# afombravo/2FAST2Q

Measured on AMD Instinct MI355X. Metric: Mreads/sec matched (150 bp, 20 bp feature, m=1), higher is better.
Workload: dtype u64 (2-bit packed bases) / u8 qualities

## Files before the change

2fast2q_amd/csrc/f2q_count_kernels.h:

```cpp
#pragma once

#define F2Q_HIST_MAX 24576u
#define F2Q_HIST_RANGE 38912u

__device__ __forceinline__ unsigned long long wave_sum(unsigned long long v)
{
    for (int o = 32; o > 0; o >>= 1) v += __shfl_down(v, o, 64);
    return v;
}

__device__ __forceinline__ void flush_stats(const Accum &acc, unsigned long long st[5], unsigned long long *lds8,
                                            unsigned long long *slab_row)
{
    const uint32_t lane = threadIdx.x & 63u;
    if (threadIdx.x < 8) lds8[threadIdx.x] = 0;
    __syncthreads();
    for (int k = 0; k < 5; k++) {
        unsigned long long v = wave_sum(st[k]);
        if (lane == 0 && v) atomicAdd(&lds8[k], v);
    }
    __syncthreads();
    if (threadIdx.x < 5) {
        unsigned long long v = lds8[threadIdx.x];
        if (slab_row) gpw(slab_row)[threadIdx.x] = v;
// ... 278 lines not shown
    unsigned long long st[5] = {0, 0, 0, 0, 0};
    auto count_hit = [&](uint32_t idx) {
        if (USE_LDS) atomicAdd(&hist[idx], 1u);
        else acc_add(&acc.counts[idx], 1ull);
    };
    auto drain = [&](bool all) {
        __builtin_amdgcn_fence(__ATOMIC_ACQ_REL, "wavefront");
        const uint32_t tail = q_tail;
        while (all ? (tail != q_head) : (tail - q_head >= 64u)) {
            if (lane < tail - q_head) {
                const unsigned long long e = queue[(q_head + lane) % F2Q_V2_QCAP];
                uint32_t idx = 0;
                const int r = packed_near_decide(run, lib, lib.mpk[(uint32_t)(e >> 62)], e & ((1ull << 62) - 1ull),
                                                 qforced[(q_head + lane) % F2Q_V2_QCAP], idx);
                if (r == R_IMPERFECT || r == R_PERFECT) { count_hit(idx); st[2]++; } else st[3]++;
            }
            q_head += (tail - q_head < 64u) ? (tail - q_head) : 64u;
        }
        __builtin_amdgcn_fence(__ATOMIC_ACQ_REL, "wavefront");
    };
    for (uint32_t base = blockIdx.x * F2Q_V2_WAVES; base < pb.n_tiles; base += gridDim.x * F2Q_V2_WAVES) {
        const uint32_t tile = base + wave;
        if (tile < pb.n_tiles) {
            int res[4]; uint64_t key[4] = {0, 0, 0, 0}; uint32_t forced[4] = {0, 0, 0, 0}, npart[4] = {0, 0, 0, 0}, lv[4];
            {
                typedef uint32_t v2 __attribute__((ext_vector_type(2)));
                v2 len2 = {pb.rmax | (pb.rmax << 16), pb.rmax | (pb.rmax << 16)};
                if (pb.len) len2 = *(const v2 F2Q_GLOBAL *)(gp(pb.len) + (uint64_t)tile * F2Q_TILE + 4u * lane);
#pragma unroll
                for (int j = 0; j < 4; j++) {
                    lv[j] = ((j < 2 ? len2.x : len2.y) >> (16 * (j & 1))) & 0xFFFFu;
                    res[j] = lv[j] == F2Q_LEN_SKIP ? R_SKIP : ((int)(lv[j] & F2Q_LEN_MASK) < need) ? R_SLOW : R_NEAR;
                }
            }
            const auto qp = gp(pb.qual) + (uint64_t)tile * pb.wq * F2Q_TILE + 4u * lane;
            const auto bp = gp(pb.bases) + (uint64_t)tile * pb.wb * F2Q_TILE + 4u * lane;
            for (int w = 0; w < W; w++) {
                const FixedGeom g = fixed_geom_of(run, w);
                U4 brow[F2Q_MAXBROWS], qrow[F2Q_MAXQROWS];
#pragma unroll
                for (int r = 0; r < F2Q_MAXBROWS; r++) {
                    uint32_t row = (uint32_t)g.bw0 + (uint32_t)(r < g.nb ? r : g.nb - 1);
                    row = row < pb.wb ? row : pb.wb - 1u;
                    brow[r] = ld_u4<true>(bp + (uint64_t)row * F2Q_TILE);
                }
#pragma unroll
                for (int r = 0; r < F2Q_MAXQROWS; r++) {
                    uint32_t row = (uint32_t)g.qw0 + (uint32_t)(r < g.nq ? r : g.nq - 1);
                    row = row < pb.wq ? row : pb.wq - 1u;
                    qrow[r] = ld_u4<true>(qp + (uint64_t)row * F2Q_TILE);
                }
                uint32_t bad[4] = {0, 0, 0, 0};
                if (g.add_hi) {
#pragma unroll
                    for (int r = 0; r < F2Q_MAXQROWS; r++)
                        if (r < g.nq) fixed4_qrow(g, r, qrow[r], bad);
                }
#pragma unroll
                for (int j = 0; j < 4; j++) {
                    if (res[j] != R_NEAR || bad[j]) continue;
                    key[j] |= fixed4_key(g, brow, j) << (2u * (uint32_t)L * npart[j]);
                    if (lv[j] & F2Q_LEN_FLAG) forced[j] |= fixed4_flags(g, qrow, j) << ((uint32_t)L * npart[j]);
                    npart[j]++;
                }
            }
#pragma unroll
            for (int j = 0; j < 4; j++) {
                if (res[j] == R_SLOW) {
                    unsigned long long st2[5] = {0, 0, 0, 0, 0};
                    const Accum acc2 = acc; const PackedBlock pb2 = pb;
                    multi_slow(runp, libp, &acc2, &pb2, tile, 4u * lane + (uint32_t)j, (int)(lv[j] & F2Q_LEN_MASK), st2);
#pragma unroll
                    for (int k = 0; k < 5; k++) st[k] += st2[k];
                    res[j] = R_SKIP;
                } else if (res[j] == R_NEAR) {
                    st[0]++;
                    if (npart[j] == 0u) { res[j] = R_QFAIL; st[4]++; }
                    else if (forced[j]) res[j] = (!do_near || __popc(forced[j]) > run.miss) ? R_NONALIGNED : R_FORCED;
                }
            }
            for (int k = W; k >= 1; k--) {
                bool mine[4]; bool any = false;
#pragma unroll
                for (int j = 0; j < 4; j++) { mine[j] = res[j] == R_NEAR && npart[j] == (uint32_t)k; any |= mine[j]; }
                if (__ballot(any) == 0ull) continue;
                const PackedGroup &pk = lib.mpk[k - 1];
                const PackedPiece ex = pk.exact;
                const uint32_t ib = pk.ib, exm = (1u << ex.bits) - 1u;
                const uint64_t imask = (1ull << ib) - 1ull;
                if (pk.len == 0u) continue;
                uint32_t s[4];
#pragma unroll
                for (int j = 0; j < 4; j++) s[j] = packed_start(key[j], ex.bits);
                while (mine[0] | mine[1] | mine[2] | mine[3]) {
                    uint64_t v0[4], v1[4];
#pragma unroll
                    for (int j = 0; j < 4; j++)
                        if (mine[j]) { const Slot2 pr = packed_pair(ptab, ex.off + s[j]); v0[j] = pr.a; v1[j] = pr.b; }
#pragma unroll
                    for (int j = 0; j < 4; j++) {
                        if (!mine[j]) continue;
                        if (v0[j] == KEY_EMPTY) mine[j] = false;
                        else if ((v0[j] >> ib) == key[j]) { mine[j] = false; res[j] = R_PERFECT; count_hit((uint32_t)(v0[j] & imask)); }
                        else if (v1[j] == KEY_EMPTY) mine[j] = false;
                        else if ((v1[j] >> ib) == key[j]) { mine[j] = false; res[j] = R_PERFECT; count_hit((uint32_t)(v1[j] & imask)); }
                        else s[j] = (s[j] + 2u) & exm;
                    }
                }
            }
            uint32_t npush = 0;
#pragma unroll
            for (int j = 0; j < 4; j++) {
                if (res[j] == R_NEAR) { if (do_near) npush++; else res[j] = R_NONALIGNED; }
                else if (res[j] == R_FORCED) npush++;
                st[1] += (res[j] == R_PERFECT); st[3] += (res[j] == R_NONALIGNED);
            }
            {
                const unsigned long long b0 = __ballot(npush & 1u), b1 = __ballot(npush & 2u), b2 = __ballot(npush & 4u);
                uint32_t at = q_tail + __builtin_amdgcn_mbcnt_hi((uint32_t)(b0 >> 32), __builtin_amdgcn_mbcnt_lo((uint32_t)b0, 0u))
                              + 2u * __builtin_amdgcn_mbcnt_hi((uint32_t)(b1 >> 32), __builtin_amdgcn_mbcnt_lo((uint32_t)b1, 0u))
                              + 4u * __builtin_amdgcn_mbcnt_hi((uint32_t)(b2 >> 32), __builtin_amdgcn_mbcnt_lo((uint32_t)b2, 0u));
                q_tail += (uint32_t)__popcll(b0) + 2u * (uint32_t)__popcll(b1) + 4u * (uint32_t)__popcll(b2);
#pragma unroll
                for (int j = 0; j < 4; j++)
                    if (res[j] == R_NEAR || res[j] == R_FORCED) {
                        queue[at % F2Q_V2_QCAP] = key[j] | ((unsigned long long)(npart[j] - 1u) << 62);
                        qforced[at % F2Q_V2_QCAP] = forced[j];
                        at++;
                    }
            }
        }
        if (do_near) drain(false);
    }
    if (do_near) drain(true);
    __shared__ unsigned long long st_lds[8];
    flush_stats(acc, st, st_lds, acc.stat_slab ? acc.stat_slab + (uint64_t)blockIdx.x * 8u : nullptr);
    if (USE_LDS) {
        __syncthreads();
        auto row = gpw(acc.slab) + (uint64_t)blockIdx.x * nf;
        for (uint32_t i = tid; i < nf; i += F2Q_V2_THREADS) row[i] = hist[i];
    }
}

#define F2Q_LT_THREADS 1024
#define F2Q_LT_WAVES (F2Q_LT_THREADS / 64)

__device__ __forceinline__ U2 lds_u2(const uint32_t *p)
{
    typedef uint32_t v2 __attribute__((ext_vector_type(2)));
    const v2 v = *reinterpret_cast<const v2 *>(p);
    return U2{v.x, v.y};
}

__device__ __forceinline__ void lt_count(uint32_t *cnt, uint32_t slot, const Accum &acc, const LtDesc &lt)
{
    const uint32_t sh = (slot & 1u) << 4;
    const uint32_t old = atomicAdd(&cnt[slot >> 1], 1u << sh);
    if (((old >> sh) & 0xFFFFu) == 0x7FFFu) {
        atomicSub(&cnt[slot >> 1], 0x8000u << sh);
        acc_add(&acc.counts[gp(lt.feat_of)[slot]], 0x8000ull);
    }
}

template <int NQ, int NB, bool NEAR, bool A20, bool MW = false>
__global__ __launch_bounds__(F2Q_LT_THREADS) void k_count_fixed4_lds(const RunDev *__restrict__ runp,
                                                                     const LibDev *__restrict__ libp, PackedBlock pb,
                                                                     Accum acc)
{
    extern __shared__ uint32_t lt_smem[];
    constexpr uint32_t NT = NEAR ? 2u : 1u;
    uint32_t *tg = lt_smem;
    uint32_t *cnt = lt_smem + NT * F2Q_LT_SLOTS;
    const RunDev &run = *runp;
    const LibDev &lib = *libp;
    LtDesc lt = lib.lt;
    if (A20) { lt.hb0 = 20u; lt.hb1 = 20u; lt.len = 20u; }
    const uint32_t nf = lib.n_features;
    const uint32_t tid = threadIdx.x, lane = tid & 63u, wave = tid >> 6;
    {
        typedef uint32_t v4 __attribute__((ext_vector_type(4)));
        const v4 F2Q_GLOBAL *src = (const v4 F2Q_GLOBAL *)gp(lt.tags);
        v4 *dst = reinterpret_cast<v4 *>(tg);
        for (uint32_t i = tid; i < NT * F2Q_LT_SLOTS / 4u; i += F2Q_LT_THREADS) dst[i] = src[i];
        for (uint32_t i = tid; i < F2Q_LT_BUCKETS; i += F2Q_LT_THREADS) cnt[i] = 0;
    }
    __syncthreads();
    FixedGeom g = MW ? fixed_geom_at(0, run.n_iter * run.length, run.thr) : fixed_geom(run);
    if (A20) { g.L = 20; g.nq = 5; g.nb = 2; g.sh = 0; g.qm_first = 0x80808080u; g.qm_last = 0x80808080u; g.kmask = (1ull << 40) - 1ull; }
    const int need = g.st + g.L;
    uint32_t w_reads = 0, w_perfect = 0, w_imperfect = 0, w_qfail = 0;
    constexpr int QR = NQ ? NQ : F2Q_MAXQROWS, BR = NB ? NB : F2Q_MAXBROWS;
    constexpr bool PIPE = NQ != 0;

    struct Rows { U4 b[BR], q[QR]; uint32_t len01, len23; };
    const uint64_t q_stride = (uint64_t)pb.wq * F2Q_TILE, b_stride = (uint64_t)pb.wb * F2Q_TILE;
    const auto q_base = gp(pb.qual) + (uint64_t)g.qw0 * F2Q_TILE + 4u * lane;
    const auto b_base = gp(pb.bases) + (uint64_t)g.bw0 * F2Q_TILE + 4u * lane;
    const auto l_base = gp(pb.len) + 4u * lane;
    auto request_tile = [&](Rows &r, uint32_t t) {
        const auto qp = q_base + (uint64_t)t * q_stride;
        const auto bp = b_base + (uint64_t)t * b_stride;
#pragma unroll
        for (int i = 0; i < BR; i++) r.b[i] = ld_u4<true>(bp + (NB ? i : (i < g.nb ? i : g.nb - 1)) * F2Q_TILE);
#pragma unroll
        for (int i = 0; i < QR; i++) r.q[i] = ld_u4<true>(qp + (NQ ? i : (i < g.nq ? i : g.nq - 1)) * F2Q_TILE);
        typedef uint32_t v2 __attribute__((ext_vector_type(2)));
        const v2 lv = __builtin_nontemporal_load((const v2 F2Q_GLOBAL *)(l_base + (uint64_t)t * F2Q_TILE));
        r.len01 = lv.x; r.len23 = lv.y;
    };
    auto decide_tile = [&](const Rows &r) {
        uint32_t bad[4] = {0, 0, 0, 0};
        bool part_fail[4] = {false, false, false, false};
        if (MW && g.add_hi) {
#pragma unroll
            for (int j = 0; j < 4; j++) {
                const int pv = mw_part_verdict(fixed4_failbits(g, r.q, j), run.n_iter, run.length);
                bad[j] = pv == 2 ? 1u : 0u; part_fail[j] = pv == 1;
            }
        } else if (g.add_hi) {
            if (A20) {
#pragma unroll
                for (int i = 0; i < QR; i++) {
#pragma unroll
                    for (int j = 0; j < 4; j++) {
                        const uint32_t w = u4get(r.q[i], j) & 0x7F7F7F7Fu;
                        bad[j] |= (w + g.add_lo) & ~(w + g.add_hi);
                    }
                }
#pragma unroll
                for (int j = 0; j < 4; j++) bad[j] &= 0x80808080u;
            } else {
#pragma unroll
                for (int i = 0; i < QR; i++)
                    if (NQ || i < g.nq) fixed4_qrow(g, i, r.q[i], bad);
            }
        }
#pragma unroll
        for (int jp = 0; jp < 4; jp += 2) {
            LtProbe q[2]; U2 e[2][4]; uint32_t forced[2]; bool cand[2];
#pragma unroll
            for (int a = 0; a < 2; a++) {
                const int j = jp + a;
                const uint32_t l = ((j < 2 ? r.len01 : r.len23) >> (16 * (j & 1))) & 0xFFFFu;
                const bool live = l != F2Q_LEN_SKIP, qf = live && bad[j] != 0u;
                cand[a] = live && !qf && (int)(l & F2Q_LEN_MASK) >= need && !(MW && part_fail[j]);
                w_reads += (uint32_t)__popcll(__ballot(live));
                w_qfail += (uint32_t)__popcll(__ballot(qf));
                forced[a] = 0;
                if ((l & F2Q_LEN_FLAG) && cand[a]) forced[a] = fixed4_flags(g, r.q, j);
                uint64_t key = fixed4_key(g, r.b, j);
                if (MW && lt.mix) { key = mw_mix(key, lt.mix); if (forced[a]) forced[a] = mw_mix_mask(forced[a], lt.mix); }
                q[a] = lt_probe(lt, key);
#pragma unroll
                for (int k = 0; k < (NEAR ? 4 : 2); k++) e[a][k] = lds_u2(tg + (uint32_t)(k >> 1) * F2Q_LT_SLOTS + 2u * q[a].b[k]);
                if (!NEAR) { e[a][2] = U2{F2Q_LT_EMPTY, F2Q_LT_EMPTY}; e[a][3] = e[a][2]; }
            }
#pragma unroll
            for (int a = 0; a < 2; a++) {
                const LtVerdict v = lt_decide<NEAR>(lt, q[a], e[a], forced[a], [&](uint32_t bk) { return lds_u2(tg + 2u * bk); });
                const LtPred cm = LT_P(cand[a]), perfect = v.perfect & cm, imperfect = v.imperfect & cm;
                if (LT_TRUE(perfect | imperfect)) lt_count(cnt, v.slot, acc, lt);
                w_perfect += (uint32_t)__popcll(perfect);
                w_imperfect += (uint32_t)__popcll(imperfect);
            }
        }
    };

    const uint32_t stride = gridDim.x * F2Q_LT_WAVES;
    uint32_t tile = blockIdx.x * F2Q_LT_WAVES + wave;
    const uint32_t last = pb.n_tiles - 1u;
    if (PIPE) {
        Rows ra, rb;
        if (tile < pb.n_tiles) {
            request_tile(ra, tile);
            for (;;) {
                __builtin_amdgcn_sched_barrier(0);
                request_tile(rb, min(tile + stride, last));
                __builtin_amdgcn_sched_barrier(0);
                decide_tile(ra);
                tile += stride;
                if (tile >= pb.n_tiles) break;
                __builtin_amdgcn_sched_barrier(0);
                request_tile(ra, min(tile + stride, last));
                __builtin_amdgcn_sched_barrier(0);
                decide_tile(rb);
                tile += stride;
                if (tile >= pb.n_tiles) break;
            }
        }
    } else {
        for (; tile < pb.n_tiles; tile += stride) { Rows r; request_tile(r, tile); decide_tile(r); }
    }
    __syncthreads();
    {
        auto row = gpw(acc.slab) + (uint64_t)blockIdx.x * nf;
        for (uint32_t i = tid; i < nf; i += F2Q_LT_THREADS) {
            const uint32_t s = gp(lt.slot_of)[i];
            row[i] = (cnt[s >> 1] >> ((s & 1u) << 4)) & 0xFFFFu;
        }
    }
    __syncthreads();
    const bool l0 = lane == 0;
    unsigned long long stv[5] = {l0 ? w_reads : 0u, l0 ? w_perfect : 0u, l0 ? w_imperfect : 0u,
                                 l0 ? w_reads - w_perfect - w_imperfect - w_qfail : 0u, l0 ? w_qfail : 0u};
    flush_stats(acc, stv, reinterpret_cast<unsigned long long *>(lt_smem), acc.stat_slab + (uint64_t)blockIdx.x * 8u);
}

__global__ __launch_bounds__(F2Q_V2_THREADS) void k_extract_fixed4(const RunDev *__restrict__ runp, EcDev ec, PackedBlock pb,
                                                                    Accum acc, uint64_t read_base)
{
    const RunDev &run = *runp;
    const uint32_t tid = threadIdx.x, lane = tid & 63u, wave = tid >> 6;
    const FixedGeom g = fixed_geom(run);
    unsigned long long st[5] = {0, 0, 0, 0, 0};
    uint32_t n_new = 0;
    for (uint32_t base = blockIdx.x * F2Q_V2_WAVES; base < pb.n_tiles; base += gridDim.x * F2Q_V2_WAVES) {
        const uint32_t tile = base + wave;
        if (tile >= pb.n_tiles) continue;
        U4 brow[F2Q_MAXBROWS], qrow[F2Q_MAXQROWS];
        const auto qp = gp(pb.qual) + (uint64_t)tile * pb.wq * F2Q_TILE + 4u * lane;
        const auto bp = gp(pb.bases) + (uint64_t)tile * pb.wb * F2Q_TILE + 4u * lane;
#pragma unroll
        for (int r = 0; r < F2Q_MAXBROWS; r++) {
            uint32_t row = (uint32_t)g.bw0 + (uint32_t)(r < g.nb ? r : (g.nb > 0 ? g.nb - 1 : 0));
            row = row < pb.wb ? row : pb.wb - 1u;
            brow[r] = ld_u4<true>(bp + (uint64_t)row * F2Q_TILE);
        }
#pragma unroll
        for (int r = 0; r < F2Q_MAXQROWS; r++) {
            const uint32_t want = (uint32_t)g.qw0 + (uint32_t)(r < g.nq ? r : (g.nq > 0 ? g.nq - 1 : 0));
            const uint32_t row = want < pb.wq ? want : pb.wq - 1u;
            qrow[r] = want < pb.wq ? ld_u4<true>(qp + (uint64_t)row * F2Q_TILE) : U4{0, 0, 0, 0};
        }
        uint32_t len01 = 0, len23 = 0;
        if (pb.len) {
            typedef uint32_t v2 __attribute__((ext_vector_type(2)));
            v2 lv = *(const v2 F2Q_GLOBAL *)(gp(pb.len) + (uint64_t)tile * F2Q_TILE + 4u * lane);
            len01 = lv.x; len23 = lv.y;
        }
        uint32_t bad[4] = {0, 0, 0, 0};
        if (g.add_hi) {
#pragma unroll
            for (int r = 0; r < F2Q_MAXQROWS; r++)
                if (r < g.nq) fixed4_qrow(g, r, qrow[r], bad);
        }
#pragma unroll
        for (int j = 0; j < 4; j++) {
            const uint32_t l = pb.len ? (((j < 2 ? len01 : len23) >> (16 * (j & 1))) & 0xFFFFu) : pb.rmax;
            if (l == F2Q_LEN_SKIP) continue;
            st[0]++;
            if (bad[j]) { st[4]++; continue; }
            const uint64_t slot = (uint64_t)tile * F2Q_TILE + 4u * lane + (uint32_t)j;
            n_new += ec64_insert_word(ec, fixed4_ec_word(g, brow, qrow, j, l), read_base + pb.first_index + (pb.index ? (uint64_t)gp(pb.index)[slot] : slot));
            st[1]++;
        }
    }
    ec64_report_new(ec, n_new);
    __shared__ unsigned long long st_lds[8];
    flush_stats(acc, st, st_lds, nullptr);
}

#define F2Q_AN_THREADS 256
#define F2Q_AN_WAVES (F2Q_AN_THREADS / 64)
#define F2Q_AN_QCAP 512u

__device__ __noinline__ void anchor_slow(const RunDev *run, const LibDev *lib, const EcDev *ec, const Accum *acc,
                                         const PackedBlock *pb, uint32_t tile, uint32_t slot, int r,
                                         unsigned long long read_index, unsigned long long *st, bool lower = false)
{
    uint8_t seq[F2Q_ANCHOR_MAXLEN], qual[F2Q_ANCHOR_MAXLEN];
    const uint32_t nw = pb->planar_nw;
    const auto bp = gp(pb->bases) + (uint64_t)tile * pb->wb * F2Q_TILE + slot;
    const auto qp = gp(pb->qual) + (uint64_t)tile * pb->wq * F2Q_TILE + slot;
    if (r > F2Q_ANCHOR_MAXLEN) r = F2Q_ANCHOR_MAXLEN;
    for (int i = 0; i < r; i++) {
        const uint32_t lo = bp[(uint64_t)(i >> 5) * F2Q_TILE], hi = bp[(uint64_t)(nw + (i >> 5)) * F2Q_TILE];
        seq[i] = (uint8_t)"ACGT"[((lo >> (i & 31)) & 1u) | (((hi >> (i & 31)) & 1u) << 1)];
        qual[i] = (uint8_t)((qp[(uint64_t)planar_qword((uint32_t)i) * F2Q_TILE] >> (8 * planar_qbyte((uint32_t)i))) & 0xFFu);
        if (qual[i] & 0x80u) { seq[i] = lower ? (uint8_t)(seq[i] | 0x20u) : (uint8_t)'N'; qual[i] &= 0x7Fu; }
    }
    general_read<const uint8_t *>(*run, *lib, *ec, *acc, seq, r, qual, r, read_index, st);
}

template <int NW, int KB, bool EC, bool USE_LDS, bool SAMEQ>
__global__ __launch_bounds__(F2Q_AN_THREADS) void k_count_anchor(const RunDev *__restrict__ runp,
                                                                  const LibDev *__restrict__ libp, EcDev ec,
                                                                  PackedBlock pb, Accum acc, uint64_t read_base)
{
    constexpr int NQW = 8 * NW;
    extern __shared__ unsigned long long smem64[];
    unsigned long long *queue = smem64 + (threadIdx.x >> 6) * F2Q_AN_QCAP;
    uint32_t *qforced = reinterpret_cast<uint32_t *>(smem64 + F2Q_AN_WAVES * F2Q_AN_QCAP) + (threadIdx.x >> 6) * F2Q_AN_QCAP;
    uint32_t *hist = reinterpret_cast<uint32_t *>(smem64 + F2Q_AN_WAVES * F2Q_AN_QCAP) + F2Q_AN_WAVES * F2Q_AN_QCAP;
    const RunDev &run = *runp;
    const LibDev &lib = *libp;
    const uint32_t nf = lib.n_features;
    const uint32_t tid = threadIdx.x, lane = tid & 63u;
    if (USE_LDS && !EC) for (uint32_t i = tid; i < nf; i += F2Q_AN_THREADS) hist[i] = 0;
    __syncthreads();
    uint32_t q_head = 0, q_tail = 0;
    const bool do_near = run.miss > 0;
    const int pk_len = (int)lib.pk.len;
    const uint32_t ah_w = phred_add_hi(run.thr), ah_u = phred_add_hi(run.thr_up), ah_d = phred_add_hi(run.thr_down);
    unsigned long long st[5] = {0, 0, 0, 0, 0};
    uint32_t n_new = 0;
#ifdef F2Q_STAMP
    unsigned long long tp[6] = {0, 0, 0, 0, 0, 0}, t0_, t1_;
#define STAMP(i) do { __builtin_amdgcn_sched_barrier(0); t1_ = __builtin_amdgcn_s_memtime(); __builtin_amdgcn_s_waitcnt(0xC07F); tp[i] += t1_ - t0_; t0_ = t1_; __builtin_amdgcn_sched_barrier(0); } while (0)
#else
#define STAMP(i) do {} while (0)
#endif

    auto count_hit = [&](uint32_t idx) {
        if (USE_LDS) atomicAdd(&hist[idx], 1u);
        else acc_add(&acc.counts[idx], 1ull);
    };

    uint32_t nLO[NW], nHI[NW], nQ[NQW], nl = F2Q_LEN_SKIP;
    auto request_tile = [&](uint32_t t) {
        const auto bpn = gp(pb.bases) + (uint64_t)t * pb.wb * F2Q_TILE + tid;
        const auto qpn = gp(pb.qual) + (uint64_t)t * pb.wq * F2Q_TILE + tid;
        nl = pb.len ? gp(pb.len)[(uint64_t)t * F2Q_TILE + tid] : pb.rmax;
#pragma unroll
        for (int w = 0; w < NW; w++) {
            nLO[w] = __builtin_nontemporal_load(bpn + (uint64_t)w * F2Q_TILE);
            nHI[w] = __builtin_nontemporal_load(bpn + (uint64_t)(NW + w) * F2Q_TILE);
        }
#pragma unroll
        for (int i = 0; i < NQW; i++) nQ[i] = __builtin_nontemporal_load(qpn + (uint64_t)i * F2Q_TILE);
    };
    if (blockIdx.x < pb.n_tiles) request_tile(blockIdx.x);
    for (uint32_t tile = blockIdx.x; tile < pb.n_tiles; tile += gridDim.x) {
#ifdef F2Q_STAMP
        __builtin_amdgcn_sched_barrier(0); t0_ = __builtin_amdgcn_s_memtime(); __builtin_amdgcn_s_waitcnt(0xC07F);
#endif
        const uint32_t l = nl;
        uint32_t LO[NW], HI[NW], Q[NQW];
#pragma unroll
        for (int w = 0; w < NW; w++) { LO[w] = nLO[w]; HI[w] = nHI[w]; }
#pragma unroll
        for (int i = 0; i < NQW; i++) Q[i] = nQ[i];
        __builtin_amdgcn_sched_barrier(0);
        if (tile + gridDim.x < pb.n_tiles) request_tile(tile + gridDim.x);
        __builtin_amdgcn_sched_barrier(0);
        uint32_t FW[NW], FU[SAMEQ ? 1 : NW], FD[SAMEQ ? 1 : NW], FLG[NW];
// ... 934 lines not shown
```

2fast2q_amd/csrc/f2q_device.h:

```cpp
#pragma once
#include <stdint.h>

#ifndef F2Q_HD
#ifdef __HIPCC__
#define F2Q_HD __host__ __device__ __forceinline__
#else
#define F2Q_HD inline
#endif
#endif

#define F2Q_DEV_MAX_ITER 16
#define F2Q_ANCHOR_MAX 128
#define F2Q_MAX_PIECES 8
#define F2Q_REG_MAXLEN 31
#define F2Q_TILE 256
#define F2Q_LEN_SKIP 0xFFFFu
#define F2Q_LEN_FLAG 0x8000u
#define F2Q_LEN_CASE 0x4000u
#define F2Q_LEN_MASK 0x3FFFu

namespace f2q {

#if defined(__HIP_DEVICE_COMPILE__)
#define F2Q_GLOBAL __attribute__((address_space(1)))
// ... 1170 lines not shown
    lt_hash(q.h1, lt.hb1, lt.hb0, 0, q.b[2], q.cmp[2], bb1);
    lt_hash(q.h1, lt.hb1, lt.hb0, 1, q.b[3], q.cmp[3], bb1);
    return q;
}
F2Q_HD int lt_exact(const LtDesc &lt, const LtProbe &q, const U2 &e0, const U2 &e1)
{
    const uint32_t w0 = lt_tag(q.cmp[0], q.h1, lt.hb1), w1 = lt_tag(q.cmp[1], q.h1, lt.hb1);
    const bool a0 = e0.x == w0, a1 = e0.y == w0, b0 = e1.x == w1, b1 = e1.y == w1;
    const uint32_t slot = (a0 | a1) ? 2u * q.b[0] + (uint32_t)a1 : 2u * q.b[1] + (uint32_t)b1;
    return (a0 | a1 | b0 | b1) ? (int)slot : -1;
}
F2Q_HD uint32_t lt_near1(const LtDesc &lt, const LtProbe &q, const U2 (&e)[4], uint32_t forced, uint32_t &hit, uint32_t &hitw)
{
    const uint32_t l0 = lt.hb0 >> 1;
    const uint32_t f0 = forced & ((1u << l0) - 1u), f1 = forced >> l0;
    uint32_t nf = 0, keep0 = ~0u, keep1 = ~0u;
    if (forced) {
#if defined(__HIP_DEVICE_COMPILE__)
        nf = (uint32_t)__popc(forced);
#else
        nf = (uint32_t)__builtin_popcount(forced);
#endif
        const uint32_t s0 = spread16(f0), s1 = spread16(f1);
        keep0 = ~(s0 | (s0 << 1)); keep1 = ~(s1 | (s1 << 1));
    }
    uint32_t n = 0;
    hit = 0; hitw = 0;
    const uint32_t m0 = (1u << lt.hb0) - 1u, m1 = (1u << lt.hb1) - 1u;
#pragma unroll
    for (int k = 0; k < 4; k++) {
        const bool t1 = k >= 2;
        const bool open = t1 ? (f1 == 0u) : (f0 == 0u);
        const uint32_t ob = t1 ? lt.hb0 : lt.hb1, om = t1 ? m0 : m1, oq = t1 ? q.h0 : q.h1, keep = t1 ? keep0 : keep1;
#pragma unroll
        for (int i = 0; i < 2; i++) {
            const uint32_t w = i ? e[k].y : e[k].x;
            const bool same = (w >> ob) == q.cmp[k];
            const uint32_t d = ham2_32(((w ^ oq) & om) & keep) + nf;
            const bool c = open & same & (d == 1u);
            n += (uint32_t)c;
            hit = c ? (((uint32_t)t1 << 31) | (2u * q.b[k] + (uint32_t)i)) : hit;
            hitw = c ? w : hitw;
        }
    }
    return n;
}
template <class RD>
F2Q_HD uint32_t lt_slot_of_t1(const LtDesc &lt, const LtProbe &q, uint32_t hitw, RD rd)
{
    const uint32_t fh0 = hitw & ((1u << lt.hb0) - 1u);
    uint32_t b0, c0, b1, c1;
    lt_hash(fh0, lt.hb0, lt.hb1, 0, b0, c0); lt_hash(fh0, lt.hb0, lt.hb1, 1, b1, c1);
    const U2 e0 = rd(b0), e1 = rd(b1);
    const uint32_t w0 = lt_tag(c0, q.h1, lt.hb1), w1 = lt_tag(c1, q.h1, lt.hb1);
    const bool a1 = e0.y == w0, hit0 = (e0.x == w0) | a1, b1y = e1.y == w1;
    return hit0 ? 2u * b0 + (uint32_t)a1 : 2u * b1 + (uint32_t)b1y;
}

#if defined(__HIP_DEVICE_COMPILE__)
typedef unsigned long long LtPred;
#define LT_P(c) __ballot(c)
#define LT_TRUE(p) __builtin_amdgcn_inverse_ballot_w64(p)
#define LT_NOT(p) (~(p))
#else
typedef bool LtPred;
#define LT_P(c) (c)
#define LT_TRUE(p) (p)
#define LT_NOT(p) (!(p))
#endif
#define LT_SEL(p, a, b) (LT_TRUE(p) ? (a) : (b))

struct LtSide { uint32_t x, slot; LtPred any, multi, first; };
F2Q_HD LtSide lt_side(uint32_t want0, uint32_t want1, uint32_t limit, uint32_t b0, uint32_t b1, const U2 &e0, const U2 &e1)
{
    const uint32_t x0 = e0.x ^ want0, x1 = e0.y ^ want0, x2 = e1.x ^ want1, x3 = e1.y ^ want1;
    const LtPred s0 = LT_P(x0 < limit), s1 = LT_P(x1 < limit), s2 = LT_P(x2 < limit), s3 = LT_P(x3 < limit);
    LtSide r;
    r.x = LT_SEL(s0, x0, LT_SEL(s1, x1, LT_SEL(s2, x2, x3)));
    r.first = s0 | s1;
    r.any = r.first | s2 | s3;
    r.multi = (s0 & (s1 | s2 | s3)) | (s1 & (s2 | s3)) | (s2 & s3);
    const LtPred odd = (LT_NOT(s0) & s1) | (LT_NOT(r.first) & LT_NOT(s2));
    r.slot = 2u * LT_SEL(r.first, b0, b1) + (LT_TRUE(odd) ? 1u : 0u);
    return r;
}
struct LtVerdict { LtPred perfect, imperfect, via1; uint32_t slot; };
template <bool NEAR, bool T1SLOT = false, class RD>
F2Q_HD LtVerdict lt_decide(const LtDesc &lt, const LtProbe &q, const U2 (&e)[4], uint32_t forced, RD rd0)
{
    const uint32_t w0 = lt_tag(q.cmp[0], q.h1, lt.hb1), w1 = lt_tag(q.cmp[1], q.h1, lt.hb1);
    const LtSide a = lt_side(w0, w1, 1u << lt.hb1, q.b[0], q.b[1], e[0], e[1]);
    LtSide b = a;
    uint32_t w2 = 0, w3 = 0;
    const LtPred unforced = LT_P(forced == 0u);
    LtPred fast = LT_NOT(a.multi);
    if (!NEAR) fast = fast & unforced;
    LtPred perfect = unforced & fast & a.any & LT_P(a.x == 0u), near = perfect & LT_NOT(perfect);
    LtPred through1 = near;
    uint32_t slot = a.slot;
    if (NEAR) {
        w2 = lt_tag(q.cmp[2], q.h0, lt.hb0); w3 = lt_tag(q.cmp[3], q.h0, lt.hb0);
        b = lt_side(w2, w3, 1u << lt.hb0, q.b[2], q.b[3], e[2], e[3]);
        fast = fast & LT_NOT(b.multi);
        perfect = perfect & fast;
        const LtPred c0 = a.any & LT_P(ham2_32(a.x) == 1u), c1 = b.any & LT_P(ham2_32(b.x) == 1u);
        near = unforced & fast & LT_NOT(perfect) & (c0 ^ c1);
        LtPred via1 = near & c1;
#if defined(__HIP_DEVICE_COMPILE__)
        const bool some_forced = LT_NOT(unforced) != 0ull;
#else
        const bool some_forced = forced != 0u;
#endif
        if (some_forced) {
            const uint32_t l0 = lt.hb0 >> 1;
            const uint32_t p = forced ? lt_ctz(forced) : 0u;
            const bool in0 = p < l0;
            const uint32_t keep = ~(3u << (2u * (in0 ? p : p - l0)));
            const uint32_t xs = in0 ? b.x : a.x;
            const LtPred one = LT_P((forced & (forced - 1u)) == 0u);
            const LtPred g = LT_NOT(unforced) & one & fast & LT_P((xs & keep) == 0u) & LT_P(in0 ? LT_TRUE(b.any) : LT_TRUE(a.any));
            near = near | g;
            via1 = via1 | (g & LT_P(in0));
        }
        if (T1SLOT) { slot = LT_SEL(via1, b.slot, slot); through1 = via1; }
        else if (LT_TRUE(via1)) slot = lt_slot_of_t1(lt, q, b.x ^ LT_SEL(b.first, w2, w3), rd0);
    }
    int sres = 0;
    bool sv1 = false;
    if (!LT_TRUE(fast)) {
        sres = R_NONALIGNED;
        const int ex = forced == 0u ? lt_exact(lt, q, e[0], e[1]) : -1;
        if (ex >= 0) { sres = R_PERFECT; slot = (uint32_t)ex; }
#if defined(__HIP_DEVICE_COMPILE__)
        else if (NEAR && __popc(forced) <= 1) {
#else
        else if (NEAR && __builtin_popcount(forced) <= 1) {
#endif
            uint32_t hit = 0, hitw = 0;
            if (lt_near1(lt, q, e, forced, hit, hitw) == 1u) {
                sres = R_IMPERFECT;
                if (T1SLOT) { slot = hit & 0x7FFFFFFFu; sv1 = (hit >> 31) != 0u; }
                else slot = (hit >> 31) ? lt_slot_of_t1(lt, q, hitw, rd0) : (hit & 0x7FFFFFFFu);
            }
        }
    }
    LtVerdict v;
    v.perfect = perfect | LT_P(sres == R_PERFECT);
    v.imperfect = near | LT_P(sres == R_IMPERFECT);
    v.via1 = through1 | LT_P(sv1);
    v.slot = slot;
    return v;
}

F2Q_HD uint32_t funnel_shr(uint32_t hi, uint32_t lo, int sh)
{
#if defined(__HIP_DEVICE_COMPILE__)
    return __builtin_amdgcn_alignbit(hi, lo, (uint32_t)sh);
#else
    return sh ? ((lo >> sh) | (hi << (32 - sh))) : lo;
#endif
}
F2Q_HD int ctz32(uint32_t x)
{
#if defined(__HIP_DEVICE_COMPILE__)
    return __ffs((int)x) - 1;
#else
    return __builtin_ctz(x);
#endif
}
F2Q_HD uint32_t range_mask32(int lo, int hi)
{
    lo = lo < 0 ? 0 : lo; hi = hi > 32 ? 32 : hi;
    if (hi <= lo) return 0u;
    uint32_t upper = hi >= 32 ? ~0u : ((1u << hi) - 1u);
    return upper & (lo >= 32 ? 0u : (~0u << lo));
}

template <int NW, int KB>
F2Q_HD void anchor_step(const uint32_t (&P)[NW], int j, uint32_t (&cnt)[KB > 0 ? KB : 1][NW], uint32_t (&ovf)[NW])
{
#pragma unroll
    for (int w = 0; w < NW; w++) {
        uint32_t x = funnel_shr(w + 1 < NW ? P[w + 1] : ~0u, P[w], j);
        if (KB == 0) ovf[w] |= x;
        else {
#pragma unroll
            for (int b = 0; b < KB; b++) { uint32_t c = cnt[b][w] & x; cnt[b][w] ^= x; x = c; }
            ovf[w] |= x;
        }
    }
}

template <int NW, int KB>
F2Q_HD void anchor_step2(const uint32_t (&P)[NW], int j1, int j2, uint32_t (&cnt)[KB > 0 ? KB : 1][NW], uint32_t (&ovf)[NW])
{
#pragma unroll
    for (int w = 0; w < NW; w++) {
        const uint32_t up = w + 1 < NW ? P[w + 1] : ~0u;
        const uint32_t x1 = funnel_shr(up, P[w], j1), x2 = funnel_shr(up, P[w], j2);
        if (KB == 0) ovf[w] |= x1 | x2;
        else {
            const uint32_t c0 = cnt[0][w];
#if defined(__HIP_DEVICE_COMPILE__)
            uint32_t x = __builtin_amdgcn_bitop3_b32(c0, x1, x2, 0xE8);
            cnt[0][w] = __builtin_amdgcn_bitop3_b32(c0, x1, x2, 0x96);
#else
            uint32_t x = (c0 & x1) | (c0 & x2) | (x1 & x2);
            cnt[0][w] = c0 ^ x1 ^ x2;
#endif
#pragma unroll
            for (int b = 1; b < KB; b++) { uint32_t c = cnt[b][w] & x; cnt[b][w] ^= x; x = c; }
            ovf[w] |= x;
        }
    }
}
template <int NW, int KB>
F2Q_HD void anchor_steps(const uint32_t (&P)[NW], uint32_t m, uint32_t (&cnt)[KB > 0 ? KB : 1][NW], uint32_t (&ovf)[NW])
{
    while (m & (m - 1u)) {
        const int j1 = ctz32(m); m &= m - 1u;
        const int j2 = ctz32(m); m &= m - 1u;
        anchor_step2<NW, KB>(P, j1, j2, cnt, ovf);
    }
    if (m) anchor_step<NW, KB>(P, ctz32(m), cnt, ovf);
}

template <int NW, int KB>
F2Q_HD void anchor_compare(const uint32_t (&cnt)[KB > 0 ? KB : 1][NW], const uint32_t (&ovf)[NW], int k, uint32_t (&hit)[NW])
{
#pragma unroll
    for (int w = 0; w < NW; w++) {
        uint32_t gt = 0, eq = ~0u;
#pragma unroll
        for (int b = KB - 1; b >= 0; b--) {
            if ((k >> b) & 1) eq &= cnt[b][w];
            else { gt |= eq & cnt[b][w]; eq &= ~cnt[b][w]; }
        }
        hit[w] = ~gt & ~ovf[w];
    }
}

template <int NW, int KBU, int KBD>
F2Q_HD void anchor_hits2p(const RunDev &run, const uint32_t *up_pos, const uint32_t *down_pos,
                          const uint32_t (&LO)[NW], const uint32_t (&HI)[NW], const uint32_t (&FLG)[NW],
                          uint32_t (&hu)[NW], uint32_t (&hd)[NW])
{
    uint32_t cu[KBU > 0 ? KBU : 1][NW], ou[NW], cd[KBD > 0 ? KBD : 1][NW], od[NW];
#pragma unroll
    for (int w = 0; w < NW; w++) {
        ou[w] = 0; od[w] = 0;
#pragma unroll
        for (int b = 0; b < (KBU > 0 ? KBU : 1); b++) cu[b][w] = 0;
#pragma unroll
        for (int b = 0; b < (KBD > 0 ? KBD : 1); b++) cd[b][w] = 0;
    }
#pragma unroll
    for (int c = 0; c < 4; c++) {
        const uint32_t la = (c & 1) ? ~0u : 0u, ha = (c & 2) ? ~0u : 0u;
        uint32_t P[NW];
#pragma unroll
        for (int w = 0; w < NW; w++) P[w] = (LO[w] ^ la) | (HI[w] ^ ha) | FLG[w];
        if (run.has_up) anchor_steps<NW, KBU>(P, up_pos[c], cu, ou);
        if (run.has_down) anchor_steps<NW, KBD>(P, down_pos[c], cd, od);
    }
    anchor_compare<NW, KBU>(cu, ou, run.msu, hu);
    anchor_compare<NW, KBD>(cd, od, run.msd, hd);
}
template <int NW, int KBU, int KBD>
F2Q_HD void anchor_hits2(const RunDev &run, const uint32_t (&LO)[NW], const uint32_t (&HI)[NW], const uint32_t (&FLG)[NW],
                         uint32_t (&hu)[NW], uint32_t (&hd)[NW])
{
    anchor_hits2p<NW, KBU, KBD>(run, run.up_pos, run.down_pos, LO, HI, FLG, hu, hd);
}

template <int NW>
F2Q_HD int first_hit(const uint32_t (&hit)[NW], int from, int to)
{
    int pos = -1;
#pragma unroll
    for (int w = NW - 1; w >= 0; w--) {
        const uint32_t m = hit[w] & range_mask32(from - 32 * w, to + 1 - 32 * w);
        if (m) pos = 32 * w + ctz32(m);
    }
    return pos;
}

template <int NW>
F2Q_HD bool any_in_range(const uint32_t (&F)[NW], int a, int b)
{
    uint32_t acc = 0;
#pragma unroll
    for (int w = 0; w < NW; w++) acc |= F[w] & range_mask32(a - 32 * w, b - 32 * w);
    return acc != 0;
}

template <int NW>
F2Q_HD uint32_t plane_extract(const uint32_t (&P)[NW], int start, int L)
{
    static_assert(NW <= 16, "plane_extract: at most 16 words");
    const uint32_t sh = (uint32_t)start & 31u, wi = (uint32_t)start >> 5;
    constexpr int NV = NW <= 8 ? 8 : 16;
    uint32_t V[NV];
#pragma unroll
    for (int w = 0; w < NV; w++) V[w] = w < NW ? funnel_shr(w + 1 < NW ? P[w + 1] : 0u, P[w], sh) : 0u;
    const bool b0 = wi & 1u, b1 = wi & 2u, b2 = wi & 4u;
    const uint32_t t0 = b0 ? V[1] : V[0], t1 = b0 ? V[3] : V[2], t2 = b0 ? V[5] : V[4], t3 = b0 ? V[7] : V[6];
// ... 305 lines not shown
```

Baseline: 161,800.

## Split lookup into exact fast path and compacted wave-batched near-match pass

Each read first gets a cheap exact-match probe of the two primary buckets. Only the reads that miss or carry forced bits are compacted across the wave with ds_permute and run through the full near-match decision in dense 64-lane batches. LDS counter atomics are issued early and their overflow checks deferred (settle) so the atomic latency overlaps other work. The first tile's global loads are also issued before the LDS table fill and barrier. This cuts divergence in the expensive near-match path, but adds permute traffic, more registers and more complex bookkeeping.

```diff
diff --git a/2fast2q_amd/csrc/f2q_count_kernels.h b/2fast2q_amd/csrc/f2q_count_kernels.h
--- a/2fast2q_amd/csrc/f2q_count_kernels.h
+++ b/2fast2q_amd/csrc/f2q_count_kernels.h
@@ -454,14 +454,19 @@
     return U2{v.x, v.y};
 }
 
+__device__ __forceinline__ uint32_t lt_count_add(uint32_t *cnt, uint32_t slot)
+{
+    return atomicAdd(&cnt[slot >> 1], 1u << ((slot & 1u) << 4));
+}
+__device__ __forceinline__ bool lt_count_passed(uint32_t old, uint32_t slot) { return ((old >> ((slot & 1u) << 4)) & 0xFFFFu) == 0x7FFFu; }
+__device__ __forceinline__ void lt_count_handoff(uint32_t *cnt, uint32_t slot, const Accum &acc, const LtDesc &lt)
+{
+    atomicSub(&cnt[slot >> 1], 0x8000u << ((slot & 1u) << 4));
+    acc_add(&acc.counts[gp(lt.feat_of)[slot]], 0x8000ull);
+}
 __device__ __forceinline__ void lt_count(uint32_t *cnt, uint32_t slot, const Accum &acc, const LtDesc &lt)
 {
-    const uint32_t sh = (slot & 1u) << 4;
-    const uint32_t old = atomicAdd(&cnt[slot >> 1], 1u << sh);
-    if (((old >> sh) & 0xFFFFu) == 0x7FFFu) {
-        atomicSub(&cnt[slot >> 1], 0x8000u << sh);
-        acc_add(&acc.counts[gp(lt.feat_of)[slot]], 0x8000ull);
-    }
+    if (lt_count_passed(lt_count_add(cnt, slot), slot)) lt_count_handoff(cnt, slot, acc, lt);
 }
 
 template <int NQ, int NB, bool NEAR, bool A20, bool MW = false>
@@ -478,15 +483,8 @@
     LtDesc lt = lib.lt;
     if (A20) { lt.hb0 = 20u; lt.hb1 = 20u; lt.len = 20u; }
     const uint32_t nf = lib.n_features;
-    const uint32_t tid = threadIdx.x, lane = tid & 63u, wave = tid >> 6;
-    {
-        typedef uint32_t v4 __attribute__((ext_vector_type(4)));
-        const v4 F2Q_GLOBAL *src = (const v4 F2Q_GLOBAL *)gp(lt.tags);
-        v4 *dst = reinterpret_cast<v4 *>(tg);
-        for (uint32_t i = tid; i < NT * F2Q_LT_SLOTS / 4u; i += F2Q_LT_THREADS) dst[i] = src[i];
-        for (uint32_t i = tid; i < F2Q_LT_BUCKETS; i += F2Q_LT_THREADS) cnt[i] = 0;
-    }
-    __syncthreads();
+    const uint32_t tid = threadIdx.x, lane = tid & 63u;
+    const uint32_t wave = (uint32_t)__builtin_amdgcn_readfirstlane((int)(tid >> 6));
     FixedGeom g = MW ? fixed_geom_at(0, run.n_iter * run.length, run.thr) : fixed_geom(run);
     if (A20) { g.L = 20; g.nq = 5; g.nb = 2; g.sh = 0; g.qm_first = 0x80808080u; g.qm_last = 0x80808080u; g.kmask = (1ull << 40) - 1ull; }
     const int need = g.st + g.L;
@@ -510,6 +508,19 @@
         const v2 lv = __builtin_nontemporal_load((const v2 F2Q_GLOBAL *)(l_base + (uint64_t)t * F2Q_TILE));
         r.len01 = lv.x; r.len23 = lv.y;
     };
+    uint32_t pend_old[4] = {0, 0, 0, 0}, pend_slot[4] = {0, 0, 0, 0}, n_pend = 0;
+    auto settle = [&]() {
+        bool any = false;
+#pragma unroll
+        for (int k = 0; k < 4; k++)
+            if ((uint32_t)k < n_pend) any |= lt_count_passed(pend_old[k], pend_slot[k]);
+        if (any) {
+#pragma unroll
+            for (int k = 0; k < 4; k++)
+                if ((uint32_t)k < n_pend && lt_count_passed(pend_old[k], pend_slot[k])) lt_count_handoff(cnt, pend_slot[k], acc, lt);
+        }
+        n_pend = 0;
+    };
     auto decide_tile = [&](const Rows &r) {
         uint32_t bad[4] = {0, 0, 0, 0};
         bool part_fail[4] = {false, false, false, false};
@@ -537,44 +548,89 @@
                     if (NQ || i < g.nq) fixed4_qrow(g, i, r.q[i], bad);
             }
         }
-#pragma unroll
-        for (int jp = 0; jp < 4; jp += 2) {
-            LtProbe q[2]; U2 e[2][4]; uint32_t forced[2]; bool cand[2];
-#pragma unroll
-            for (int a = 0; a < 2; a++) {
-                const int j = jp + a;
-                const uint32_t l = ((j < 2 ? r.len01 : r.len23) >> (16 * (j & 1))) & 0xFFFFu;
-                const bool live = l != F2Q_LEN_SKIP, qf = live && bad[j] != 0u;
-                cand[a] = live && !qf && (int)(l & F2Q_LEN_MASK) >= need && !(MW && part_fail[j]);
-                w_reads += (uint32_t)__popcll(__ballot(live));
-                w_qfail += (uint32_t)__popcll(__ballot(qf));
-                forced[a] = 0;
-                if ((l & F2Q_LEN_FLAG) && cand[a]) forced[a] = fixed4_flags(g, r.q, j);
-                uint64_t key = fixed4_key(g, r.b, j);
-                if (MW && lt.mix) { key = mw_mix(key, lt.mix); if (forced[a]) forced[a] = mw_mix_mask(forced[a], lt.mix); }
-                q[a] = lt_probe(lt, key);
-#pragma unroll
-                for (int k = 0; k < (NEAR ? 4 : 2); k++) e[a][k] = lds_u2(tg + (uint32_t)(k >> 1) * F2Q_LT_SLOTS + 2u * q[a].b[k]);
-                if (!NEAR) { e[a][2] = U2{F2Q_LT_EMPTY, F2Q_LT_EMPTY}; e[a][3] = e[a][2]; }
-            }
-#pragma unroll
-            for (int a = 0; a < 2; a++) {
-                const LtVerdict v = lt_decide<NEAR>(lt, q[a], e[a], forced[a], [&](uint32_t bk) { return lds_u2(tg + 2u * bk); });
-                const LtPred cm = LT_P(cand[a]), perfect = v.perfect & cm, imperfect = v.imperfect & cm;
-                if (LT_TRUE(perfect | imperfect)) lt_count(cnt, v.slot, acc, lt);
-                w_perfect += (uint32_t)__popcll(perfect);
-                w_imperfect += (uint32_t)__popcll(imperfect);
-            }
+        LtProbe0 p[4]; U2 e0[4], e1[4]; uint32_t klo[4], khi[4], forced[4]; bool cand[4];
+#pragma unroll
+        for (int j = 0; j < 4; j++) {
+            const uint32_t l = ((j < 2 ? r.len01 : r.len23) >> (16 * (j & 1))) & 0xFFFFu;
+            const bool live = l != F2Q_LEN_SKIP, qf = live && bad[j] != 0u;
+            cand[j] = live && !qf && (int)(l & F2Q_LEN_MASK) >= need && !(MW && part_fail[j]);
+            w_reads += (uint32_t)__popcll(__ballot(live));
+            w_qfail += (uint32_t)__popcll(__ballot(qf));
+            forced[j] = 0;
+            if ((l & F2Q_LEN_FLAG) && cand[j]) forced[j] = fixed4_flags(g, r.q, j);
+            uint64_t key = fixed4_key(g, r.b, j);
+            if (MW && lt.mix) { key = mw_mix(key, lt.mix); if (forced[j]) forced[j] = mw_mix_mask(forced[j], lt.mix); }
+            p[j] = lt_probe0(lt, key);
+            e0[j] = lds_u2(tg + 2u * p[j].b0);
+            e1[j] = lds_u2(tg + 2u * p[j].b1);
+            klo[j] = (uint32_t)key; khi[j] = lt_rec_hi(key, forced[j]);
+        }
+        LtExact x[4];
+#pragma unroll
+        for (int j = 0; j < 4; j++) x[j] = lt_exact_stage(p[j], e0[j], e1[j], cand[j], forced[j]);
+        settle();
+#pragma unroll
+        for (int j = 0; j < 4; j++) {
+            pend_old[j] = 0;
+            if (x[j].hit) pend_old[j] = lt_count_add(cnt, x[j].slot);
+            pend_slot[j] = x[j].slot;
+            w_perfect += (uint32_t)__popcll(__ballot(x[j].hit));
+        }
+        n_pend = 4;
+        if (!NEAR) return;
+        uint32_t pre[5], pos[4];
+        pre[0] = 0;
+#pragma unroll
+        for (int j = 0; j < 4; j++) {
+            const unsigned long long m = __ballot(x[j].batch);
+            pos[j] = pre[j] + __builtin_amdgcn_mbcnt_hi((uint32_t)(m >> 32), __builtin_amdgcn_mbcnt_lo((uint32_t)m, 0u));
+            pre[j + 1] = pre[j] + (uint32_t)__popcll(m);
+        }
+        for (uint32_t lo = 0; lo < pre[4]; lo += 64u) {
+            const uint32_t at = lo + lane;
+            uint32_t rlo = 0, rhi = 0;
+#pragma unroll
+            for (int j = 0; j < 4; j++) {
+                if (!lt_batch_has(pre, j, lo)) continue;
+                const bool send = x[j].batch && pos[j] - lo < 64u;
+                const int to = (int)(4u * (send ? pos[j] - lo : lt_dump(pre, j, lo)));
+                const uint32_t a = (uint32_t)__builtin_amdgcn_ds_permute(to, (int)klo[j]);
+                const uint32_t b = (uint32_t)__builtin_amdgcn_ds_permute(to, (int)khi[j]);
+                const bool mine = at >= pre[j] && at < pre[j + 1];
+                rlo = mine ? a : rlo; rhi = mine ? b : rhi;
+            }
+            const bool valid = at < pre[4];
+            const LtProbe q = lt_probe(lt, lt_rec_key(rlo, rhi));
+            U2 e[4];
+#pragma unroll
+            for (int k = 0; k < 4; k++) e[k] = lds_u2(tg + (uint32_t)(k >> 1) * F2Q_LT_SLOTS + 2u * q.b[k]);
+            const LtVerdict v = lt_decide<NEAR>(lt, q, e, lt_rec_forced(rhi), [&](uint32_t bk) { return lds_u2(tg + 2u * bk); });
+            settle();
+            const LtPred cm = LT_P(valid), perfect = v.perfect & cm, imperfect = v.imperfect & cm;
+            pend_old[0] = 0;
+            if (LT_TRUE(perfect | imperfect)) pend_old[0] = lt_count_add(cnt, v.slot);
+            pend_slot[0] = v.slot;
+            n_pend = 1;
+            w_perfect += (uint32_t)__popcll(perfect);
+            w_imperfect += (uint32_t)__popcll(imperfect);
         }
     };
 
     const uint32_t stride = gridDim.x * F2Q_LT_WAVES;
     uint32_t tile = blockIdx.x * F2Q_LT_WAVES + wave;
     const uint32_t last = pb.n_tiles - 1u;
+    Rows ra, rb;
+    if (PIPE && tile < pb.n_tiles) request_tile(ra, tile);
+    {
+        typedef uint32_t v4 __attribute__((ext_vector_type(4)));
+        const v4 F2Q_GLOBAL *src = (const v4 F2Q_GLOBAL *)gp(lt.tags);
+        v4 *dst = reinterpret_cast<v4 *>(tg);
+        for (uint32_t i = tid; i < NT * F2Q_LT_SLOTS / 4u; i += F2Q_LT_THREADS) dst[i] = src[i];
+        for (uint32_t i = tid; i < F2Q_LT_BUCKETS; i += F2Q_LT_THREADS) cnt[i] = 0;
+    }
+    __syncthreads();
     if (PIPE) {
-        Rows ra, rb;
         if (tile < pb.n_tiles) {
-            request_tile(ra, tile);
             for (;;) {
                 __builtin_amdgcn_sched_barrier(0);
                 request_tile(rb, min(tile + stride, last));
@@ -593,6 +649,7 @@
     } else {
         for (; tile < pb.n_tiles; tile += stride) { Rows r; request_tile(r, tile); decide_tile(r); }
     }
+    settle();
     __syncthreads();
     {
         auto row = gpw(acc.slab) + (uint64_t)blockIdx.x * nf;
diff --git a/2fast2q_amd/csrc/f2q_device.h b/2fast2q_amd/csrc/f2q_device.h
--- a/2fast2q_amd/csrc/f2q_device.h
+++ b/2fast2q_amd/csrc/f2q_device.h
@@ -1346,6 +1346,37 @@
     return v;
 }
 
+struct LtProbe0 { uint32_t b0, b1, w0, w1; };
+F2Q_HD LtProbe0 lt_probe0(const LtDesc &lt, uint64_t key)
+{
+    const uint32_t h0 = (uint32_t)key & ((1u << lt.hb0) - 1u), h1 = (uint32_t)(key >> lt.hb0);
+    LtProbe0 p;
+    uint32_t c0, c1;
+    lt_hash(h0, lt.hb0, lt.hb1, 0, p.b0, c0);
+    lt_hash(h0, lt.hb0, lt.hb1, 1, p.b1, c1);
+    p.w0 = lt_tag(c0, h1, lt.hb1); p.w1 = lt_tag(c1, h1, lt.hb1);
+    return p;
+}
+struct LtExact { bool hit, batch; uint32_t slot; };
+F2Q_HD LtExact lt_exact_stage(const LtProbe0 &p, const U2 &e0, const U2 &e1, bool cand, uint32_t forced)
+{
+    const bool a0 = e0.x == p.w0, a1 = e0.y == p.w0, b0 = e1.x == p.w1, b1 = e1.y == p.w1;
+    LtExact r;
+    r.hit = cand && forced == 0u && (a0 | a1 | b0 | b1);
+    r.batch = cand && !r.hit;
+    r.slot = (a0 | a1) ? 2u * p.b0 + (uint32_t)a1 : 2u * p.b1 + (uint32_t)b1;
+    return r;
+}
+F2Q_HD uint32_t lt_rec_hi(uint64_t key, uint32_t forced) { return (uint32_t)(key >> 32) | (forced << 10); }
+F2Q_HD uint64_t lt_rec_key(uint32_t lo, uint32_t hi) { return ((uint64_t)(hi & 0x3FFu) << 32) | lo; }
+F2Q_HD uint32_t lt_rec_forced(uint32_t hi) { return hi >> 10; }
+F2Q_HD uint32_t lt_dump(const uint32_t (&pre)[5], int j, uint32_t lo)
+{
+    const uint32_t s = (pre[j] > lo ? pre[j] : lo) - lo, e = pre[j + 1] - lo < 64u ? pre[j + 1] - lo : 64u;
+    return e < 64u ? e : (s ? s - 1u : 0u);
+}
+F2Q_HD bool lt_batch_has(const uint32_t (&pre)[5], int j, uint32_t lo) { return pre[j] < lo + 64u && pre[j + 1] > lo; }
+
 F2Q_HD uint32_t funnel_shr(uint32_t hi, uint32_t lo, int sh)
 {
 #if defined(__HIP_DEVICE_COMPILE__)
```

New measurement: 170,900 (median of 6 runs). 1.06x the previous value.
